# PRiME-project/PRiMEStereoMatch

Hardware: AMD Instinct MI355X
Metric: cost-volume voxels/s (CVC+CVF+WTA) (higher is better)
Workload: dtype f32; 1 GPU; synthetic 1920x1080 pair, D=256, float32 (BASELINE configs[3]); W=1920, H=1080, D=256, parallelism=1 GPU, kernel_variant=0, lr_check_on_gpu=False, batch=1, ranks=1, same_device=False, frames_in_flight=1

## Files before the change

primestereomatch_amd/csrc/psm_api_filter.cpp:

```cpp
#include "psm_ctx.h"

#include <cstring>
#include <utility>

using namespace psm;

namespace psm {

int ensure_vol(psm_ctx *c, int side)
{
    if (c->vol[side]) return 0;
    const size_t V = (size_t)c->W * c->H * c->Dloc;
    PSM_HIP(c, hipMalloc(&c->vol[side], V * velem(c)));
    return 0;
}

int ensure_ab(psm_ctx *c)
{
    if (c->ab) return 0;
    const size_t V = (size_t)c->W * c->H * c->Dloc;
    PSM_HIP(c, hipMalloc((void **)&c->ab, V * sizeof(float4)));
    return 0;
}

// ... 117 lines not shown
    sp.maps = c->Dloc == c->D && !sp.two_phase;
    sp.scratch_bytes = 2 * pc_plan_select(m, c->W, c->H, sp.n1, PC_PLANES, npairs, batch).scratch_bytes();
    return sp;
}

int enqueue_select(psm_ctx *c, const PcPairs &P, const SelPlan &sp)
{
    const bool u8 = c->dtype == PSM_U8;
    {
        Prof p(c, PSM_K_CVF_F);
        launch_cvf_select2(c->stream, c->march, P, u8, c->W, c->H, sp.n1, c->d0, next_pc_stamp(c), sp.two_phase ? 1 : 0, sp.S);
    }
    if (sp.maps && !P.tab && maps_writable(c)) return 1;
    {
        Prof p(c, PSM_K_WTA);
        launch_chunk_min2sides(c->stream, c->march, P, c->W, c->H, sp.n1, sp.maps);
    }
    if (sp.n2 > 0) {
        Prof p(c, PSM_K_CVF_F);
        launch_cvf_select_keys2(c->stream, c->march, P, u8, c->W, c->H, sp.n2, c->d0, next_pc_stamp(c), 2, sp.S);
    }
    return 0;
}

int adopt_staged_pair(psm_ctx *c)
{
    if (c->next_depth < 0) return 0;
    bool ok = true;
    if (c->range_next_pending) {
        PSM_HIP(c, hipEventSynchronize(c->ev_up));
        ok = range_inside(c, 1, -PSM_IMG_EXP, PSM_IMG_EXP);
// ... 267 lines not shown
```

primestereomatch_amd/csrc/psm_kernels.h:

```cpp
#pragma once
#include <hip/hip_runtime.h>
#include <stdint.h>

namespace psm {

struct Guidance {
    float4 *g1;
    float4 *g2;
    float4 *g3;
    float2 *g4;
};

struct March {
    int seg_rows;
    int waves;
    int flags;
    int dstep = 1;
    int inflight = 1;
    int ybeg = 0, yend = 0;
    int y0(int H) const { (void)H; return yend > ybeg ? ybeg : 0; }
    int y1(int H) const { return yend > ybeg ? yend : H; }
    int rows(int H) const { return y1(H) - y0(H); }
};

// ... 34 lines not shown
    bool narrow;
    size_t rec_per_chunk;
    int rec_bytes;
    size_t scratch_bytes() const { return rec_per_chunk * (size_t)nchunks * rec_bytes; }
};
PcPlan pc_plan(int W, int rows, int Dloc, int seg_rows_opt, int form, int batch = 1, int inflight = 1);
PcPlan pc_plan_select(March m, int W, int H, int Dloc, int form, int npairs, bool batch);
int pc_seed_stride(int W, int rows, bool u8);
constexpr int PC_TS_SLOTS = 4096;
void launch_cvf_select(hipStream_t s, March m, const float *vin, Guidance g, int W, int H, int Dloc, const float4 *g1_other,
                       int d_begin, int cvc_mode, void *scratch, unsigned long long *ts = nullptr, const uint8_t *p4_own = nullptr,
                       const uint8_t *p4_other = nullptr);
void launch_chunk_min(hipStream_t s, March m, int W, int H, int Dloc, void *scratch, long long *keys, uint8_t *map);
void launch_cvf_select2(hipStream_t s, March m, const PcPairs &P, bool u8, int W, int H, int Dloc, int d_begin, unsigned long long *ts,
                        int sel, int step);
void launch_chunk_min2sides(hipStream_t s, March m, const PcPairs &P, int W, int H, int Dloc, bool to_maps);
void launch_cvf_select_keys2(hipStream_t s, March m, const PcPairs &P, bool u8, int W, int H, int Dloc, int d_begin,
                             unsigned long long *ts, int sel, int step);
void launch_box8(hipStream_t s, int variant, March m, const float *vol, float *out, int W, int H, int Dloc);
void launch_wta(hipStream_t s, const float *vol, int W, int H, int d_begin, int Dloc, long long *keys,
                uint8_t *map);
void launch_merge(hipStream_t s, const long long *keys_all, size_t rank_stride, int nranks, int n,
                  uint8_t *map);
void launch_lr_check(hipStream_t s, const uint8_t *l, const uint8_t *r, int W, int H, uint8_t *lv,
                     uint8_t *rv);

void launch_fill_inv(hipStream_t s, uint8_t *dis, const uint8_t *valid, size_t side, int W, int H);

void launch_wgt_median(hipStream_t s, uint8_t *dis, const uint8_t *valid, const float4 *g1, int W, int H, int maxDis, int right,
                       int *nxt, int *prog, int *err);
constexpr int WM_LANE_MIN = 8192;
// ... 161 lines not shown
```

primestereomatch_amd/csrc/psm_pc.hip:

```cpp
#include "psm_kernels.h"
#include "psm_cost.h"
#include "psm_dev.h"
#include "../../include/primesm_hip.h"

#include <mutex>
#include <type_traits>

#include "psm_pc_debug.inc"

namespace psm {

typedef float f4v __attribute__((ext_vector_type(4)));

constexpr int PC_RING = 4;

template <int MODE, bool NARROW = false> struct PcLayout;
template <> struct PcLayout<0, false> { static constexpr int NA = 2, NB = 2, OUT_A = 52, OUT_B = 48, COLS = 96; };
template <> struct PcLayout<1, false> { static constexpr int NA = 2, NB = 2, OUT_A = 57, OUT_B = 54, COLS = 107; };
template <> struct PcLayout<2, false> : PcLayout<1, false> {};
template <> struct PcLayout<1, true> { static constexpr int NA = 1, NB = 1, OUT_A = 57, OUT_B = 50, COLS = 50; };
template <> struct PcLayout<2, true> : PcLayout<1, true> {};
constexpr int PC_K_LD_AUX = 0;
constexpr int PC_KEY_LD_AUX = 1;

// ... 25 lines not shown
typedef unsigned pc_u3 __attribute__((ext_vector_type(3)));
__device__ __forceinline__ float3 pc_load3(__amdgpu_buffer_rsrc_t r, int voff, int soff)
{
    const pc_u3 v = __builtin_amdgcn_raw_buffer_load_b96(r, voff, soff, 0);
    return make_float3(__uint_as_float(v.x), __uint_as_float(v.y), __uint_as_float(v.z));
}

struct PcSide {
    const float4 *G1, *G2, *G3;
    const float2 *G4;
    const float4 *Gother;
    float *kcost;
    unsigned *kdisp;
};

struct PcSel {
    int sel, step;
    int nxcd;
    int spread;
    int n;
    unsigned long long rec_total;
    int dstep;
};
__device__ __forceinline__ int pc_slice(const PcSel &o, int i)
{
    if (o.spread > 1) {
        int r = 0, base = 0;
        for (; r < o.spread; ++r) {
            const int cnt = (o.n - r + o.spread - 1) / o.spread;
            if (i < base + cnt) break;
            base += cnt;
        }
        i = (i - base) * o.spread + r;
    }
    return o.sel == 1 ? i * o.step : (o.sel == 2 ? (i / (o.step - 1)) * o.step + i % (o.step - 1) + 1 : i);
}

template <bool VEC4, int CVC, int MODE, bool U8 = false, bool BATCH = false, int VAR = 0, bool NARROW = false>
__global__ __launch_bounds__(64 * (PcLayout<MODE, NARROW>::NA + PcLayout<MODE, NARROW>::NB))
__attribute__((amdgpu_waves_per_eu(MODE == 2 ? 4 : 1, MODE == 2 ? 4 : 8)))
void k_cvf_pc(
    const float *__restrict__ vin, float *__restrict__ vout, const float4 *__restrict__ G1a, const float4 *__restrict__ G2a,
    const float4 *__restrict__ G3a, const float2 *__restrict__ G4a, int W, int H, int Dloc, int ngroups, int nsegs, int seg_rows,
    int ybeg, int yend, const float4 *__restrict__ Gothera, int d_begin, int DC, float *__restrict__ kcosta, unsigned *__restrict__ kdispa, int nbmax,
    PcSide side1, PcSel dyn, unsigned long long *__restrict__ ts, const PcPair *__restrict__ batch)
{
    constexpr bool TOL = VAR == 1, FMA = VAR == 2;
    static_assert(VAR >= 0 && VAR <= 2 && !(TOL && (U8 || MODE == 0)) && !(FMA && (U8 || BATCH)), "tolerance form: float select forms; FMA solve: float mode, single pair");
    if constexpr (BATCH) {
        static_assert(CVC == 3 && MODE != 0, "batched launches: both volumes per launch, select forms");
// ... 16 lines not shown
    const float4 *const G1 = s1 ? side1.G1 : G1a, *const G2 = s1 ? side1.G2 : G2a, *const G3 = s1 ? side1.G3 : G3a;
    const float2 *const G4 = s1 ? side1.G4 : G4a;
    const float4 *const Gother = s1 ? side1.Gother : Gothera;
    float *const kcost = s1 ? side1.kcost : kcosta;
    unsigned *const kdisp = s1 ? side1.kdisp : kdispa;
    static_assert(!NARROW || (MODE != 0 && CVC == 3), "the narrow layout exists for the two-volume select forms");
    using L = PcLayout<MODE, NARROW>;
    constexpr int PC_NA = L::NA, PC_NB = L::NB, PC_OUT_A = L::OUT_A, PC_OUT_B = L::OUT_B, PC_COLS = L::COLS;
    constexpr int PC_MCOLS = PC_NA * PC_OUT_A;
    constexpr bool SCALED = MODE != 0;
    constexpr float QSCALE = SCALED ? 0x1p-12f : 1.0f;
#define PSM_BOX(N) (SCALED ? (float)(N) : box_out(N))
    static_assert(PC_MCOLS >= PC_COLS + 7 && PC_OUT_A <= 57 && PC_OUT_B <= 57 && (MODE != 0 || (PC_COLS % 4) == 0), "bad producer/consumer layout");
    __shared__ __attribute__((aligned(16))) float4 ring[PC_RING][4][PC_MCOLS];
    __shared__ __attribute__((aligned(16))) float qbuf[MODE == 0 ? 2 : 1][MODE == 0 ? 4 : 1][MODE == 0 ? PC_COLS : 4];
    const int nchunks = (Dloc + DC - 1) / DC;
    int id = blockIdx.x;
    const int npairs = ngroups * nsegs;
    const int nitems = npairs * nchunks;
    const int ipx = (nitems + dyn.nxcd - 1) / dyn.nxcd;
    const int xcd = id % dyn.nxcd, jj = id / dyn.nxcd;
    const int item = xcd * ipx + jj;
    if (jj >= ipx || item >= nitems) return;
    if (ts != nullptr && threadIdx.x == 0) {
        (void)__hip_atomic_fetch_min(ts, (unsigned long long)wall_clock64(), __ATOMIC_RELAXED, __HIP_MEMORY_SCOPE_AGENT);
        if (blockIdx.x == 0 && blockIdx.y == 0) ts[2 * PC_TS_SLOTS] = (unsigned long long)MODE;
    }
    const int pair = item / nchunks, ch = item % nchunks;
    const int g = pair % ngroups, seg = pair / ngroups;
    const int wave = __builtin_amdgcn_readfirstlane(threadIdx.x >> 6), lane = threadIdx.x & 63;
    const bool is_a = wave < PC_NA;
    const int xg = g * PC_COLS;
    const int xm0 = xg - 4;
    const int y0 = ybeg + seg * seg_rows, y1 = min(yend, y0 + seg_rows);
    const int mstart = max(0, y0 - 4);
    const int mend = min(H - 1, max(y1 + 2, 4 - y0));
    const int nbA = (mend - mstart + 1 + 3) >> 2;
    const int nf = (y1 - y0) + 7;
    const int nbB = (nf + 3) >> 2;
    const int iters = nbB + 3;
    const int i1 = ((lane + 1) & 63) << 2, i2 = ((lane + 2) & 63) << 2, i4 = ((lane + 4) & 63) << 2;
    (void)i1;
    const size_t HW = (size_t)H * W;

    PC_TRACE_BEGIN()
    const int nds = MODE == 1 ? min(DC, Dloc - ch * DC) : 1;
    bool first = true;
    int rb = 0;
    for (int ds = 0; ds < nds; ++ds) {
    const int d = ch * DC + ds;
    const bool last_slice = ds == nds - 1;
    if (is_a) {
        const int xa0 = xm0 + wave * PC_OUT_A;
        const int ci = r101c(xa0 - 4 + lane, W);
        const int xa = xa0 + lane;
        const int xac = xa < 0 ? 0 : (xa > W - 1 ? W - 1 : xa);
        const bool mvalid = lane < PC_OUT_A;
        const float *vd = vin + (size_t)pc_slice(dyn, d) * HW;
        const int dg = d_begin + dyn.dstep * pc_slice(dyn, d);
        const bool inb = right ? (ci < W - dg) : (ci >= dg);
        const int cpart = right ? min(ci + dg, W - 1) : max(ci - dg, 0);
        const bool any_border = CVC != 0 && __builtin_amdgcn_ballot_w64(!inb) != 0;
        VTree t0 = {}, t1 = {}, t2 = {}, t3 = {};
        float pin[2];
        float4 oth[2], gin[2], o2[2], o3[2];
        float2 o4[2];
        constexpr bool LEANA = MODE == 2;
        const __amdgpu_buffer_rsrc_t rG1 = pc_rsrc(G1, (unsigned)HW * 16u), rG2 = pc_rsrc(G2, (unsigned)HW * 16u);
        const __amdgpu_buffer_rsrc_t rG3 = pc_rsrc(G3, (unsigned)HW * 16u), rG4 = pc_rsrc(G4, (unsigned)HW * 8u);
        const __amdgpu_buffer_rsrc_t rGo = pc_rsrc(CVC == 0 ? G1 : Gother, (unsigned)HW * 16u);
        const __amdgpu_buffer_rsrc_t rV = pc_rsrc(CVC == 0 ? (const void *)vd : (const void *)G1, (unsigned)HW * 4u);
        const __amdgpu_buffer_rsrc_t rPo = pc_rsrc(U8 ? (s1 ? (const void *)vin : (const void *)vout) : (const void *)G1, (unsigned)HW * 4u);
        unsigned po[2];
        const int vci = ci * 16, vcp = cpart * 16, vxa = xac * 16;
// ... 88 lines not shown
        for (int b = nbA; b < (last_slice ? iters : nbB); ++b) PC_SYNC();
#undef PSM_STEP_PA
#undef PSM_ISSUE_PA
#undef PSM_ISSUE_PIX
#undef PSM_ISSUE_GUI
#undef PSM_ISSUE_PA2
    } else {
        const int wb = wave - PC_NA;
        const int bwidth = wb < PC_NB - 1 ? PC_OUT_B : PC_COLS - (PC_NB - 1) * PC_OUT_B;
        const int xb0 = xg + wb * PC_OUT_B;
        const int xmod = xb0 - 4 + lane;
        int mc = r101(xmod, W) - xm0;
        mc = mc < 0 ? 0 : (mc > PC_MCOLS - 1 ? PC_MCOLS - 1 : mc);
        const int xb = xb0 + lane;
        const int xbc = min(xb, W - 1);
        float *od = vout + (MODE == 0 ? (size_t)pc_slice(dyn, d) * HW : 0);
        const int amax = 4 * nbA - 1;
        VTree t0 = {}, t1 = {}, t2 = {}, t3 = {};
        float o1x[4], o1y[4], o1z[4];
        const size_t krec = (size_t)(ch * npairs + pair) * nbmax * PC_COLS + wb * PC_OUT_B;
        const __amdgpu_buffer_rsrc_t rKc = pc_rsrc(MODE == 1 ? (const void *)(reinterpret_cast<float4 *>(kcost) + krec) : (const void *)G1, (unsigned)nbmax * PC_COLS * 16u);
        const __amdgpu_buffer_rsrc_t rKd = pc_rsrc(MODE == 1 ? (const void *)(kdisp + krec) : (const void *)G1, (unsigned)nbmax * PC_COLS * 4u);
#define PSM_K_LOAD(C)                                                                              \
    {                                                                                              \
        const pc_u4 v_ = __builtin_amdgcn_raw_buffer_load_b128(rKc, lane * 16, (C) * (PC_COLS * 16), PC_K_LD_AUX); \
        kq = make_float4(__uint_as_float(v_.x), __uint_as_float(v_.y), __uint_as_float(v_.z), __uint_as_float(v_.w)); \
        kd4 = __builtin_amdgcn_raw_buffer_load_b32(rKd, lane * 4, (C) * (PC_COLS * 4), PC_K_LD_AUX); \
    }
        float4 kq = make_float4(__builtin_inff(), __builtin_inff(), __builtin_inff(), __builtin_inff());
        unsigned kd4 = 0;
        long long *const keyp = reinterpret_cast<long long *>(kcost);
        const __amdgpu_buffer_rsrc_t rKy = pc_rsrc(MODE == 2 ? (const void *)keyp : (const void *)G1, (unsigned)HW * 8u);
        long long kcur[4] = {0, 0, 0, 0};
#define PSM_KEY_LOAD1(SLOT, J)                                            \
    {                                                                                              \
        int yk_ = y0 + (J) - 7;                                                                    \
        yk_ = yk_ < 0 ? 0 : (yk_ > H - 1 ? H - 1 : yk_);                                           \
        const pc_u2 v_ = __builtin_amdgcn_raw_buffer_load_b64(rKy, xbc * 8, yk_ * W * 8, PC_KEY_LD_AUX); \
        kcur[SLOT] = (long long)(((unsigned long long)v_.y << 32) | v_.x);                         \
    }
        const __amdgpu_buffer_rsrc_t rG1 = pc_rsrc(G1, (unsigned)HW * 16u);
        const int vxb = xbc * 16;
        const int dg = d_begin + dyn.dstep * pc_slice(dyn, d);
        const bool lane_out = lane < bwidth && xb < W;
#define PSM_ISSUE_PB(SLOT, J)                                                           \
    {                                                                                   \
        int yb_ = y0 + (J) - 7;                                                         \
        yb_ = yb_ < 0 ? 0 : (yb_ > H - 1 ? H - 1 : yb_);                                \
        const float3 g_ = pc_load3(rG1, vxb, yb_ * W * 16);                             \
        o1x[SLOT] = g_.x; o1y[SLOT] = g_.y; o1z[SLOT] = g_.z;                           \
    }
        auto model_of = [&](int J) -> const float4 * {
            int a = r101(y0 - 4 + J, H) - mstart;
            a = a < 0 ? 0 : (a > amax ? amax : a);
            return &ring[((a >> 2) + rb) & (PC_RING - 1)][a & 3][mc];
        };
        auto store_batch = [&](int c) {
            if constexpr (MODE == 0) {
// ... 15 lines not shown
                            if (xg + cc < W) row[cc] = src[cc];
                    }
                }
            }
            }
        };
        constexpr bool LEANB = MODE == 2;
        PSM_ISSUE_PB(0, 0) PSM_ISSUE_PB(1, 1)
        if (!LEANB) { PSM_ISSUE_PB(2, 2) PSM_ISSUE_PB(3, 3) }
        if constexpr (MODE == 1) {
            if (!first) {
                PSM_K_LOAD(0)
            }
        }
        if constexpr (MODE == 2) { PSM_KEY_LOAD1(0, 0) PSM_KEY_LOAD1(1, 1) }
        if (ds == 0) {
            PC_SYNC();
            PC_SYNC();
        }
        auto batch_b = [&](const int c) __attribute__((always_inline)) {
            if (c >= 1) store_batch(c - 1);
            {
                const int j0 = 4 * c;
                float4 a_cur = *model_of(j0), a_nxt;
                float qv[4];
#define PSM_STEP_PB(K)                                                                              \
    {                                                                                               \
        if (K < 3) a_nxt = *model_of(j0 + K + 1);      \
        double h0 = hsum8<TOL>(a_cur.x, i1, i2, i4);                                                \
        double h1 = hsum8<TOL>(a_cur.y, i1, i2, i4);                                                \
        double h2 = hsum8<TOL>(a_cur.z, i1, i2, i4);                                                \
// ... 56 lines not shown
#undef PSM_K_LOAD
    }
    if (MODE == 1) __builtin_amdgcn_s_waitcnt(0);
    first = false;
    rb = (rb + nbA) & (PC_RING - 1);
    }
#undef PSM_BOX
    if (ts != nullptr && threadIdx.x == 0)
        (void)__hip_atomic_fetch_max(ts + PC_TS_SLOTS, (unsigned long long)wall_clock64(), __ATOMIC_RELAXED, __HIP_MEMORY_SCOPE_AGENT);
    PC_TRACE_END()
}

__global__ __launch_bounds__(256) void k_chunk_min(const float4 *kcost, const unsigned *kdisp, int nchunks, int npairs,
                                                  int nbmax, int ngroups, int seg_rows, int W, int H, long long *keys,
                                                  uint8_t *map, const float4 *__restrict__ kcost1, const unsigned *__restrict__ kdisp1,
                                                  int ybeg, int yend, const PcPair *__restrict__ batch, int to_maps, int cols)
{
    if (batch) {
        const PcPair pp = batch[blockIdx.z];
        const size_t rec_total = (size_t)npairs * nbmax * cols * nchunks;
        kcost = (const float4 *)pp.scratch;
        kdisp = (const unsigned *)(kcost + rec_total);
        kcost1 = (const float4 *)((const char *)pp.scratch + rec_total * 20);
        kdisp1 = (const unsigned *)(kcost1 + rec_total);
        keys = pp.keys;
        map = to_maps ? pp.maps : nullptr;
    }
    if (blockIdx.y == 1) {
        kcost = kcost1;
        kdisp = kdisp1;
        if (keys) keys += (size_t)W * H;
        if (map) map += (size_t)W * H;
    }
    const size_t nrec = (size_t)npairs * nbmax * cols;
    const size_t idx = (size_t)blockIdx.x * blockDim.x + threadIdx.x;
    if (idx >= nrec) return;
    const int col = (int)(idx % cols);
    size_t t = idx / cols;
    const int c = (int)(t % nbmax);
    const int pair = (int)(t / nbmax);
    const int g = pair % ngroups, seg = pair / ngroups;
    const int x = g * cols + col;
    if (x >= W) return;
    const int y0 = ybeg + seg * seg_rows, y1 = min(yend, y0 + seg_rows);
    const int ya = y0 + 4 * c - 7;
    if (ya + 3 < y0 || ya >= y1) return;
    float4 kc = kcost[idx];
    unsigned kd = kdisp[idx];
    long long best[4] = {pack_key_f32(kc.x, kd & 0xff), pack_key_f32(kc.y, (kd >> 8) & 0xff), pack_key_f32(kc.z, (kd >> 16) & 0xff),
                         pack_key_f32(kc.w, kd >> 24)};
    for (int ch = 1; ch < nchunks; ++ch) {
        kc = kcost[(size_t)ch * nrec + idx];
        kd = kdisp[(size_t)ch * nrec + idx];
        const long long k0 = pack_key_f32(kc.x, kd & 0xff), k1 = pack_key_f32(kc.y, (kd >> 8) & 0xff),
                        k2 = pack_key_f32(kc.z, (kd >> 16) & 0xff), k3 = pack_key_f32(kc.w, kd >> 24);
        best[0] = k0 < best[0] ? k0 : best[0];
        best[1] = k1 < best[1] ? k1 : best[1];
        best[2] = k2 < best[2] ? k2 : best[2];
        best[3] = k3 < best[3] ? k3 : best[3];
    }
#pragma unroll
    for (int k = 0; k < 4; ++k) {
        const int yo = ya + k;
        if (yo < y0 || yo >= y1) continue;
        const size_t o = (size_t)yo * W + x;
        if (keys) keys[o] = best[k];
        if (map) map[o] = (uint8_t)((unsigned long long)best[k] & 0xffull);
    }
// ... 16 lines not shown
    int dev = 0;
    if (hipGetDevice(&dev) != hipSuccess || dev < 0 || dev >= 64) dev = 0;
    std::lock_guard<std::mutex> lock(mu);
    PcDev &d = cache[dev];
    if (d.nxcd == 0) {
        int nx = 0, cus = 0;
        if (hipDeviceGetAttribute(&nx, hipDeviceAttributeNumberOfXccs, dev) != hipSuccess || nx < 1) nx = 1;
        if (hipDeviceGetAttribute(&cus, hipDeviceAttributeMultiprocessorCount, dev) != hipSuccess || cus < 1) cus = 256;
        (void)hipGetLastError();
        d.cus_per_xcd = cus / nx > 0 ? cus / nx : 1;
        d.nxcd = nx;
    }
    return d;
}


PcPlan pc_plan(int W, int rows, int Dloc, int seg_rows_opt, int form, int batch, int inflight)
{
    const bool planes = (form & 3) == PC_PLANES, keys = (form & 3) == PC_KEYS;
    if (PSM_KNOB(planes ? "PSM_PC_SEGP" : "PSM_PC_SEGK", 0) > 0 && (planes || keys))
        seg_rows_opt = PSM_KNOB(planes ? "PSM_PC_SEGP" : "PSM_PC_SEGK", 0);
    const int sides = ((form & PC_BOTH) ? 2 : 1) * (batch > 1 ? batch : 1);
    const PcDev dev = pc_dev();
    PcPlan pl;
    pl.nxcd = dev.nxcd;
    constexpr int WIDE = PcLayout<1>::COLS, NARROW = PcLayout<1, true>::COLS;
    const bool select2 = (form & 3) != PC_STORE && (form & PC_BOTH);
    const int narrow_knob = PSM_KNOB("PSM_PC_NARROW", 0);
    pl.narrow = select2 && (narrow_knob ? narrow_knob == 1 : 2 * ((W + NARROW - 1) / NARROW) < 4 * ((W + WIDE - 1) / WIDE));
    const int cols = (form & 3) == PC_STORE ? PcLayout<0>::COLS : (pl.narrow ? NARROW : WIDE);
// ... 43 lines not shown
    pl.rec_per_chunk = (size_t)pl.ngroups * pl.nsegs * pl.nbmax * pl.cols;
    pl.rec_bytes = 20;
    return pl;
}

constexpr int PC_KEY_SPREAD = 4;

int pc_seed_stride(int W, int rows, bool u8)
{
    const int e = PSM_KNOB("PSM_PC_S", 0);
    if (e > 1) return e;
    if (rows < 200 || (u8 && (size_t)W * rows >= 1500000)) return 5;
    return 8;
}

static int pc_blocks(const PcPlan &pl, int chunks) { return pl.nxcd * ((pl.ngroups * pl.nsegs * chunks + pl.nxcd - 1) / pl.nxcd); }

struct PcArgs {
    const float *vin;
    float *vout;
    int W, H, Dloc, ybeg, yend, d_begin;
    PcSide side[2];
    PcSel sel;
    unsigned long long *ts;
    const PcPair *batch;
};

struct PcForm {
    int mode, cvc;
    bool u8;
    int var;
    bool batch, narrow, vec4;
};

template <int V> using pc_int = std::integral_constant<int, V>;
template <int... Vs, class Fn> static void pc_pick(int v, Fn &&fn) { (void)((v == Vs && (fn(pc_int<Vs>{}), true)) || ...); }
template <class Fn> static void pc_pick_bool(bool b, Fn &&fn) { if (b) fn(std::true_type{}); else fn(std::false_type{}); }

static void pc_launch(hipStream_t s, const PcPlan &pl, dim3 grid, const PcArgs &a, const PcForm &f)
{
    using F = std::false_type;
    using T = std::true_type;
    const bool planes = f.mode == PC_PLANES;
    const PcSide &s0 = a.side[0];
    auto go = [&](auto V4, auto CV, auto MD, auto U, auto BT, auto VR, auto NW) {
        using L = PcLayout<MD, NW>;
        hipLaunchKernelGGL(HIP_KERNEL_NAME(k_cvf_pc<V4, CV, MD, U, BT, VR, NW>), grid, dim3(64 * (L::NA + L::NB)), 0, s, a.vin, a.vout,
                           s0.G1, s0.G2, s0.G3, s0.G4, a.W, a.H, a.Dloc, pl.ngroups, pl.nsegs, pl.seg_rows, a.ybeg, a.yend, s0.Gother,
                           a.d_begin, planes ? pl.DC : 1, s0.kcost, s0.kdisp, planes ? pl.nbmax : 0, a.side[1], a.sel, a.ts, a.batch);
    };
    if (f.mode == PC_STORE)
        pc_pick_bool(f.vec4, [&](auto V4) { pc_pick<0, 1, 2>(f.cvc, [&](auto CV) {
            pc_pick<0, 2>(f.var, [&](auto VR) { go(V4, CV, pc_int<0>{}, F{}, F{}, VR, F{}); }); }); });
    else if (f.cvc != 3)
        pc_pick<0, 1, 2>(f.cvc, [&](auto CV) {
            if constexpr (CV != 0) if (f.u8) return go(F{}, CV, pc_int<1>{}, T{}, F{}, pc_int<0>{}, F{});
            pc_pick<0, 2>(f.var, [&](auto VR) { go(F{}, CV, pc_int<1>{}, F{}, F{}, VR, F{}); });
        });
    else
// ... 6 lines not shown

static PcSide pc_planes(const PcPlan &pl, void *scratch, int v)
{
    PcSide p = {};
    p.kcost = (float *)((char *)scratch + v * pl.scratch_bytes());
    p.kdisp = (unsigned *)(p.kcost + 4 * pl.rec_per_chunk * pl.nchunks);
    return p;
}

static int pc_var(March m, bool u8)
{
    return u8 ? 0 : (m.flags & PSM_FLAG_FMA_SOLVE) ? 2 : (m.flags & PSM_FLAG_F32_TOL) ? 1 : 0;
}

static void pc_chunk_min(hipStream_t s, March m, const PcPlan &pl, int W, int H, int sides, int npairs, void *scratch,
                         long long *keys, uint8_t *map, const PcPair *tab = nullptr, bool to_maps = false)
{
    const PcSide p0 = scratch ? pc_planes(pl, scratch, 0) : PcSide{}, p1 = scratch && sides == 2 ? pc_planes(pl, scratch, 1) : PcSide{};
    hipLaunchKernelGGL(k_chunk_min, dim3((unsigned)((pl.rec_per_chunk + 255) / 256), sides, npairs), dim3(256), 0, s,
                       (const float4 *)p0.kcost, (const unsigned *)p0.kdisp, pl.nchunks, pl.ngroups * pl.nsegs, pl.nbmax, pl.ngroups,
                       pl.seg_rows, W, H, keys, map, (const float4 *)p1.kcost, (const unsigned *)p1.kdisp, m.y0(H), m.y1(H), tab,
                       to_maps ? 1 : 0, pl.cols);
}

void launch_cvf_fused(hipStream_t s, March m, const float *vin, float *vout, Guidance gd, int W, int H, int Dloc,
                      int ybeg, int yend, const float4 *g1_other, int d_begin, int cvc_mode, unsigned long long *ts)
{
    if (yend <= ybeg) return;
    const PcPlan pl = pc_plan(W, yend - ybeg, Dloc, m.seg_rows, PC_STORE);
    PcArgs a = {vin, vout, W, H, Dloc, ybeg, yend, d_begin, {}, PcSel{0, 1, pl.nxcd, 0, Dloc, 0, 1}, ts, nullptr};
    a.side[0] = PcSide{gd.g1, gd.g2, gd.g3, gd.g4, g1_other, nullptr, nullptr};
    const int cvc = cvc_mode == 1 || cvc_mode == 2 ? cvc_mode : 0;
    pc_launch(s, pl, dim3(pc_blocks(pl, Dloc)), a, {PC_STORE, cvc, false, (m.flags & PSM_FLAG_FMA_SOLVE) ? 2 : 0, false, false, (W & 3) == 0});
}

void launch_cvf_select(hipStream_t s, March m, const float *vin, Guidance gd, int W, int H, int Dloc, const float4 *g1_other,
                       int d_begin, int cvc_mode, void *scratch, unsigned long long *ts, const uint8_t *p4_own, const uint8_t *p4_other)
{
    const PcPlan pl = pc_plan(W, m.rows(H), Dloc, m.seg_rows, PC_PLANES);
    const int cvc = cvc_mode == 1 || cvc_mode == 2 ? cvc_mode : 0;
    const bool u8 = p4_own && cvc != 0;
    PcArgs a = {u8 ? (const float *)p4_own : vin, u8 ? (float *)const_cast<uint8_t *>(p4_other) : nullptr, W, H, Dloc, m.y0(H), m.y1(H),
                d_begin, {}, PcSel{0, 1, pl.nxcd, 0, Dloc, 0, 1}, ts, nullptr};
    const PcSide k = pc_planes(pl, scratch, 0);
    a.side[0] = PcSide{gd.g1, gd.g2, gd.g3, gd.g4, g1_other, k.kcost, k.kdisp};
    pc_launch(s, pl, dim3(pc_blocks(pl, pl.nchunks)), a, {PC_PLANES, cvc, u8, (m.flags & PSM_FLAG_FMA_SOLVE) ? 2 : 0, false, false, false});
}

void launch_chunk_min(hipStream_t s, March m, int W, int H, int Dloc, void *scratch, long long *keys, uint8_t *map)
{
    pc_chunk_min(s, m, pc_plan(W, m.rows(H), Dloc, m.seg_rows, PC_PLANES), W, H, 1, 1, scratch, keys, map);
}

PcPlan pc_plan_select(March m, int W, int H, int Dloc, int form, int npairs, bool batch)
{
    return pc_plan(W, m.rows(H), Dloc, m.seg_rows, form | PC_BOTH, npairs, batch ? 1 : m.inflight);
}

static PcArgs pc_args2(March m, const PcPlan &pl, int form, const PcPairs &P, bool u8, int W, int H, int Dloc, int d_begin, PcSel sel,
                       unsigned long long *ts)
{
    PcArgs a = {nullptr, nullptr, W, H, Dloc, m.y0(H), m.y1(H), d_begin, {}, sel, ts, P.tab};
    if (P.tab) return a;
    const PcPair &p = P.one;
    if (u8) { a.vin = (const float *)p.p4[0]; a.vout = (float *)p.p4[1]; }
    for (int v = 0; v < 2; ++v) {
        const PcSide k = form == PC_PLANES ? pc_planes(pl, p.scratch, v) : PcSide{};
        a.side[v] = PcSide{p.g[v].g1, p.g[v].g2, p.g[v].g3, p.g[v].g4, p.g[v ^ 1].g1, k.kcost, k.kdisp};
        if (form == PC_KEYS) a.side[v].kcost = (float *)(p.keys + v * (size_t)W * H);
    }
    return a;
}

void launch_cvf_select2(hipStream_t s, March m, const PcPairs &P, bool u8, int W, int H, int Dloc, int d_begin, unsigned long long *ts,
                        int sel, int step)
{
    const PcPlan pl = pc_plan_select(m, W, H, Dloc, PC_PLANES, P.n, P.tab != nullptr);
    const unsigned long long rec_total = P.tab ? (unsigned long long)pl.rec_per_chunk * pl.nchunks : 0;
    const PcArgs a = pc_args2(m, pl, PC_PLANES, P, u8, W, H, Dloc, d_begin, PcSel{sel, step, pl.nxcd, 0, Dloc, rec_total, m.dstep}, ts);
    pc_launch(s, pl, dim3(pc_blocks(pl, pl.nchunks), 2, P.n), a, {PC_PLANES, 3, u8, pc_var(m, u8), P.tab != nullptr, pl.narrow, false});
}

void launch_chunk_min2sides(hipStream_t s, March m, const PcPairs &P, int W, int H, int Dloc, bool to_maps)
{
    const PcPlan pl = pc_plan_select(m, W, H, Dloc, PC_PLANES, P.n, P.tab != nullptr);
    if (P.tab) pc_chunk_min(s, m, pl, W, H, 2, P.n, nullptr, nullptr, nullptr, P.tab, to_maps);
    else pc_chunk_min(s, m, pl, W, H, 2, 1, P.one.scratch, P.one.keys, to_maps ? P.one.maps : nullptr);
}

void launch_cvf_select_keys2(hipStream_t s, March m, const PcPairs &P, bool u8, int W, int H, int Dloc, int d_begin,
                             unsigned long long *ts, int sel, int step)
{
    const PcPlan pl = pc_plan_select(m, W, H, Dloc, PC_KEYS, P.n, P.tab != nullptr);
    const PcArgs a = pc_args2(m, pl, PC_KEYS, P, u8, W, H, Dloc, d_begin,
                              PcSel{sel, step, pl.nxcd, PSM_KNOB("PSM_PC_SPREAD", PC_KEY_SPREAD), Dloc, 0, m.dstep}, ts);
    pc_launch(s, pl, dim3(pc_blocks(pl, Dloc), 2, P.n), a, {PC_KEYS, 3, u8, pc_var(m, u8), P.tab != nullptr, pl.narrow, false});
}

}
```

Baseline: 159.7 billion voxels/s.

## Skip dead disparity slices and chunks per column group in select kernels

Adds host-side liveness analysis that works out, for each column group and side, which disparity slices lie entirely outside the image border or are trivially zero. The producer/consumer select kernels and the chunk-min reduction then iterate only over live work items, with a compacted item indexing scheme and trimmed per-chunk slice ranges. This removes cost-volume filtering and reduction work for disparities that cannot affect the result. In exchange it adds index-decoding overhead in each block and falls back to full work when the live pattern is too irregular.

```diff
diff --git a/primestereomatch_amd/csrc/psm_api_filter.cpp b/primestereomatch_amd/csrc/psm_api_filter.cpp
--- a/primestereomatch_amd/csrc/psm_api_filter.cpp
+++ b/primestereomatch_amd/csrc/psm_api_filter.cpp
@@ -155,7 +155,7 @@
     if (sp.maps && !P.tab && maps_writable(c)) return 1;
     {
         Prof p(c, PSM_K_WTA);
-        launch_chunk_min2sides(c->stream, c->march, P, c->W, c->H, sp.n1, sp.maps);
+        launch_chunk_min2sides(c->stream, c->march, P, c->W, c->H, sp.n1, sp.maps, c->d0, sp.two_phase ? 1 : 0, sp.S);
     }
     if (sp.n2 > 0) {
         Prof p(c, PSM_K_CVF_F);
diff --git a/primestereomatch_amd/csrc/psm_kernels.h b/primestereomatch_amd/csrc/psm_kernels.h
--- a/primestereomatch_amd/csrc/psm_kernels.h
+++ b/primestereomatch_amd/csrc/psm_kernels.h
@@ -1,6 +1,7 @@
 #pragma once
 #include <hip/hip_runtime.h>
 #include <stdint.h>
+#include "psm_live.h"
 
 namespace psm {
 
@@ -72,7 +73,7 @@
 void launch_chunk_min(hipStream_t s, March m, int W, int H, int Dloc, void *scratch, long long *keys, uint8_t *map);
 void launch_cvf_select2(hipStream_t s, March m, const PcPairs &P, bool u8, int W, int H, int Dloc, int d_begin, unsigned long long *ts,
                         int sel, int step);
-void launch_chunk_min2sides(hipStream_t s, March m, const PcPairs &P, int W, int H, int Dloc, bool to_maps);
+void launch_chunk_min2sides(hipStream_t s, March m, const PcPairs &P, int W, int H, int Dloc, bool to_maps, int d_begin, int sel, int step);
 void launch_cvf_select_keys2(hipStream_t s, March m, const PcPairs &P, bool u8, int W, int H, int Dloc, int d_begin,
                              unsigned long long *ts, int sel, int step);
 void launch_box8(hipStream_t s, int variant, March m, const float *vol, float *out, int W, int H, int Dloc);
diff --git a/primestereomatch_amd/csrc/psm_live.h b/primestereomatch_amd/csrc/psm_live.h
--- /dev/null
+++ b/primestereomatch_amd/csrc/psm_live.h
@@ -0,0 +1,52 @@
+#pragma once
+
+#if defined(__HIPCC__)
+#define PSM_LIVE_FN __host__ __device__ inline
+#else
+#define PSM_LIVE_FN inline
+#endif
+
+namespace psm {
+
+PSM_LIVE_FN int pc_border_from(int right, int xfirst, int xlast, int W)
+{
+    if (xlast > W - 1) xlast = W - 1;
+    if (right) return (W - 1 - xfirst) + 9;
+    const int t = xlast + 7;
+    return xfirst <= 0 && t < 8 ? 8 : t;
+}
+
+PSM_LIVE_FN bool pc_dead(int right, int xfirst, int xlast, int W, int dg, int dprev)
+{
+    if (dg == 0) return true;
+    return dprev >= 0 && dprev >= pc_border_from(right, xfirst, xlast, W);
+}
+
+PSM_LIVE_FN int pc_sel_index(int sel, int step, int j)
+{
+    return sel == 1 ? j * step : (sel == 2 ? (j / (step - 1)) * step + j % (step - 1) + 1 : j);
+}
+
+struct PcOwn {
+    int on;
+    int d_begin, dstep;
+    int sel, step;
+};
+
+PSM_LIVE_FN bool pc_dead_at(const PcOwn &o, int right, int xfirst, int xlast, int W, int j)
+{
+    if (!o.on) return false;
+    const int i = pc_sel_index(o.sel, o.step, j);
+    return pc_dead(right, xfirst, xlast, W, o.d_begin + i * o.dstep, i > 0 ? o.d_begin + (i - 1) * o.dstep : -1);
+}
+
+PSM_LIVE_FN int pc_live_end(const PcOwn &o, int right, int xfirst, int xlast, int W, int n)
+{
+    if (!o.on) return n;
+    const int t = pc_border_from(right, xfirst, xlast, W);
+    const int ilim = o.d_begin >= t ? 1 : 1 + (t - o.d_begin + o.dstep - 1) / o.dstep;
+    const int below = o.sel == 1 ? (ilim + o.step - 1) / o.step : (o.sel == 2 ? ilim - (ilim + o.step - 1) / o.step : ilim);
+    return below < n ? below : n;
+}
+
+}
diff --git a/primestereomatch_amd/csrc/psm_pc.hip b/primestereomatch_amd/csrc/psm_pc.hip
--- a/primestereomatch_amd/csrc/psm_pc.hip
+++ b/primestereomatch_amd/csrc/psm_pc.hip
@@ -1,6 +1,7 @@
 #include "psm_kernels.h"
 #include "psm_cost.h"
 #include "psm_dev.h"
+#include "psm_live.h"
 #include "../../include/primesm_hip.h"
 
 #include <mutex>
@@ -63,26 +64,42 @@
     unsigned *kdisp;
 };
 
+constexpr int PC_LIVE_MAX = 6;
+struct PcLive {
+    int on;
+    int lo, full;
+    int pre[2], nshort[2], tot[2];
+    int cnt[2][PC_LIVE_MAX];
+};
+__host__ __device__ __forceinline__ int pc_live_count(const PcLive &lv, int side, int g)
+{
+    const int k = g - (side ? lv.pre[1] : lv.pre[0]), ns = side ? lv.nshort[1] : lv.nshort[0];
+    int c = lv.full;
+#pragma unroll
+    for (int i = 0; i < PC_LIVE_MAX; ++i)
+        if (i == k && i < ns) c = side ? lv.cnt[1][i] : lv.cnt[0][i];
+    return c;
+}
 struct PcSel {
     int sel, step;
     int nxcd;
     int spread;
-    int n;
     unsigned long long rec_total;
     int dstep;
+    PcLive live;
 };
-__device__ __forceinline__ int pc_slice(const PcSel &o, int i)
+__device__ __forceinline__ int pc_spread(const PcSel &o, int n, int i)
 {
     if (o.spread > 1) {
         int r = 0, base = 0;
         for (; r < o.spread; ++r) {
-            const int cnt = (o.n - r + o.spread - 1) / o.spread;
+            const int cnt = (n - r + o.spread - 1) / o.spread;
             if (i < base + cnt) break;
             base += cnt;
         }
         i = (i - base) * o.spread + r;
     }
-    return o.sel == 1 ? i * o.step : (o.sel == 2 ? (i / (o.step - 1)) * o.step + i % (o.step - 1) + 1 : i);
+    return i;
 }
 
 template <bool VEC4, int CVC, int MODE, bool U8 = false, bool BATCH = false, int VAR = 0, bool NARROW = false>
@@ -129,10 +146,11 @@
     static_assert(PC_MCOLS >= PC_COLS + 7 && PC_OUT_A <= 57 && PC_OUT_B <= 57 && (MODE != 0 || (PC_COLS % 4) == 0), "bad producer/consumer layout");
     __shared__ __attribute__((aligned(16))) float4 ring[PC_RING][4][PC_MCOLS];
     __shared__ __attribute__((aligned(16))) float qbuf[MODE == 0 ? 2 : 1][MODE == 0 ? 4 : 1][MODE == 0 ? PC_COLS : 4];
-    const int nchunks = (Dloc + DC - 1) / DC;
     int id = blockIdx.x;
     const int npairs = ngroups * nsegs;
-    const int nitems = npairs * nchunks;
+    const PcLive &lv = dyn.live;
+    const int ltot = s1 ? lv.tot[1] : lv.tot[0];
+    const int nitems = nsegs * ltot;
     const int ipx = (nitems + dyn.nxcd - 1) / dyn.nxcd;
     const int xcd = id % dyn.nxcd, jj = id / dyn.nxcd;
     const int item = xcd * ipx + jj;
@@ -141,8 +159,29 @@
         (void)__hip_atomic_fetch_min(ts, (unsigned long long)wall_clock64(), __ATOMIC_RELAXED, __HIP_MEMORY_SCOPE_AGENT);
         if (blockIdx.x == 0 && blockIdx.y == 0) ts[2 * PC_TS_SLOTS] = (unsigned long long)MODE;
     }
-    const int pair = item / nchunks, ch = item % nchunks;
-    const int g = pair % ngroups, seg = pair / ngroups;
+    const int seg = item / ltot;
+    int g, gi = item - seg * ltot, gn = lv.full;
+    {
+        const int pre = s1 ? lv.pre[1] : lv.pre[0], ns = s1 ? lv.nshort[1] : lv.nshort[0];
+        if (gi < pre * lv.full) { g = gi / lv.full; gi -= g * lv.full; }
+        else {
+            gi -= pre * lv.full;
+            g = pre;
+            bool found = false;
+#pragma unroll
+            for (int k = 0; k < PC_LIVE_MAX; ++k) {
+                const int c = s1 ? lv.cnt[1][k] : lv.cnt[0][k];
+                if (!found && k < ns) {
+                    if (gi < c) { found = true; gn = c; }
+                    else { gi -= c; ++g; }
+                }
+            }
+            if (!found) { const int q = gi / lv.full; g += q; gi -= q * lv.full; }
+        }
+    }
+    const int pair = seg * ngroups + g;
+    const int ch = lv.lo + gi;
+    const int sl0 = pc_sel_index(dyn.sel, dyn.step, MODE == 2 ? lv.lo + pc_spread(dyn, gn, gi) : ch);
     const int wave = __builtin_amdgcn_readfirstlane(threadIdx.x >> 6), lane = threadIdx.x & 63;
     const bool is_a = wave < PC_NA;
     const int xg = g * PC_COLS;
@@ -159,20 +198,26 @@
     const size_t HW = (size_t)H * W;
 
     PC_TRACE_BEGIN()
-    const int nds = MODE == 1 ? min(DC, Dloc - ch * DC) : 1;
+    int ds_lo = 0, ds_hi = MODE == 1 ? min(DC, Dloc - ch * DC) : 1;
+    if (MODE == 1 && lv.on) {
+        const PcOwn own = {1, d_begin, dyn.dstep, dyn.sel, dyn.step};
+        while (ds_lo < ds_hi && pc_dead_at(own, right, xg, xg + PC_COLS - 1, W, ch * DC + ds_lo)) ++ds_lo;
+        while (ds_hi > ds_lo && pc_dead_at(own, right, xg, xg + PC_COLS - 1, W, ch * DC + ds_hi - 1)) --ds_hi;
+        if (ds_lo >= ds_hi) return;
+    }
     bool first = true;
     int rb = 0;
-    for (int ds = 0; ds < nds; ++ds) {
-    const int d = ch * DC + ds;
-    const bool last_slice = ds == nds - 1;
+    for (int ds = ds_lo; ds < ds_hi; ++ds) {
+    const int sl = MODE == 1 ? pc_sel_index(dyn.sel, dyn.step, ch * DC + ds) : sl0;
+    const bool last_slice = ds == ds_hi - 1;
     if (is_a) {
         const int xa0 = xm0 + wave * PC_OUT_A;
         const int ci = r101c(xa0 - 4 + lane, W);
         const int xa = xa0 + lane;
         const int xac = xa < 0 ? 0 : (xa > W - 1 ? W - 1 : xa);
         const bool mvalid = lane < PC_OUT_A;
-        const float *vd = vin + (size_t)pc_slice(dyn, d) * HW;
-        const int dg = d_begin + dyn.dstep * pc_slice(dyn, d);
+        const float *vd = vin + (size_t)sl * HW;
+        const int dg = d_begin + dyn.dstep * sl;
         const bool inb = right ? (ci < W - dg) : (ci >= dg);
         const int cpart = right ? min(ci + dg, W - 1) : max(ci - dg, 0);
         const bool any_border = CVC != 0 && __builtin_amdgcn_ballot_w64(!inb) != 0;
@@ -291,7 +336,7 @@
         mc = mc < 0 ? 0 : (mc > PC_MCOLS - 1 ? PC_MCOLS - 1 : mc);
         const int xb = xb0 + lane;
         const int xbc = min(xb, W - 1);
-        float *od = vout + (MODE == 0 ? (size_t)pc_slice(dyn, d) * HW : 0);
+        float *od = vout + (MODE == 0 ? (size_t)sl * HW : 0);
         const int amax = 4 * nbA - 1;
         VTree t0 = {}, t1 = {}, t2 = {}, t3 = {};
         float o1x[4], o1y[4], o1z[4];
@@ -318,7 +363,7 @@
     }
         const __amdgpu_buffer_rsrc_t rG1 = pc_rsrc(G1, (unsigned)HW * 16u);
         const int vxb = xbc * 16;
-        const int dg = d_begin + dyn.dstep * pc_slice(dyn, d);
+        const int dg = d_begin + dyn.dstep * sl;
         const bool lane_out = lane < bwidth && xb < W;
 #define PSM_ISSUE_PB(SLOT, J)                                                           \
     {                                                                                   \
@@ -364,7 +409,7 @@
             }
         }
         if constexpr (MODE == 2) { PSM_KEY_LOAD1(0, 0) PSM_KEY_LOAD1(1, 1) }
-        if (ds == 0) {
+        if (ds == ds_lo) {
             PC_SYNC();
             PC_SYNC();
         }
@@ -451,7 +496,8 @@
 __global__ __launch_bounds__(256) void k_chunk_min(const float4 *kcost, const unsigned *kdisp, int nchunks, int npairs,
                                                   int nbmax, int ngroups, int seg_rows, int W, int H, long long *keys,
                                                   uint8_t *map, const float4 *__restrict__ kcost1, const unsigned *__restrict__ kdisp1,
-                                                  int ybeg, int yend, const PcPair *__restrict__ batch, int to_maps, int cols)
+                                                  int ybeg, int yend, const PcPair *__restrict__ batch, int to_maps, int cols,
+                                                  PcLive lv)
 {
     if (batch) {
         const PcPair pp = batch[blockIdx.z];
@@ -482,13 +528,12 @@
     const int y0 = ybeg + seg * seg_rows, y1 = min(yend, y0 + seg_rows);
     const int ya = y0 + 4 * c - 7;
     if (ya + 3 < y0 || ya >= y1) return;
-    float4 kc = kcost[idx];
-    unsigned kd = kdisp[idx];
-    long long best[4] = {pack_key_f32(kc.x, kd & 0xff), pack_key_f32(kc.y, (kd >> 8) & 0xff), pack_key_f32(kc.z, (kd >> 16) & 0xff),
-                         pack_key_f32(kc.w, kd >> 24)};
-    for (int ch = 1; ch < nchunks; ++ch) {
-        kc = kcost[(size_t)ch * nrec + idx];
-        kd = kdisp[(size_t)ch * nrec + idx];
+    const int c_lo = lv.lo, c_hi = min(nchunks, lv.lo + pc_live_count(lv, blockIdx.y == 1, g));
+    const long long none = pack_key_f32(__builtin_inff(), 0);
+    long long best[4] = {none, none, none, none};
+    for (int ch = c_lo; ch < c_hi; ++ch) {
+        const float4 kc = kcost[(size_t)ch * nrec + idx];
+        const unsigned kd = kdisp[(size_t)ch * nrec + idx];
         const long long k0 = pack_key_f32(kc.x, kd & 0xff), k1 = pack_key_f32(kc.y, (kd >> 8) & 0xff),
                         k2 = pack_key_f32(kc.z, (kd >> 16) & 0xff), k3 = pack_key_f32(kc.w, kd >> 24);
         best[0] = k0 < best[0] ? k0 : best[0];
@@ -535,6 +580,42 @@
     return d;
 }
 
+
+PcLive pc_live(int W, int cols, int ngroups, int n, int DC, bool chunks, const PcOwn &own)
+{
+    const int nu = chunks ? (n + DC - 1) / DC : n;
+    PcLive all = {};
+    all.full = nu;
+    all.tot[0] = all.tot[1] = ngroups * nu;
+    if (!own.on || n < 1 || ngroups < 1) return all;
+    PcLive lv = {};
+    lv.on = 1;
+    const int skip0 = own.d_begin == 0 && own.sel != 2 ? 1 : 0;
+    lv.lo = skip0 && (!chunks || DC == 1 || n == 1) ? 1 : 0;
+    lv.full = nu - lv.lo;
+    for (int side = 0; side < 2; ++side) {
+        int gs = -1, ge = -1;
+        for (int g = 0; g < ngroups; ++g) {
+            const int xf = g * cols, xl = xf + cols - 1;
+            const int L = pc_live_end(own, side, xf, xl, W, n);
+            if ((L < n && !pc_dead_at(own, side, xf, xl, W, L)) || (L - 1 >= skip0 && pc_dead_at(own, side, xf, xl, W, L - 1))) return all;
+            const int end = chunks ? (L + DC - 1) / DC : L, c = L > skip0 && end > lv.lo ? end - lv.lo : 0;
+            lv.tot[side] += c;
+            if (c == lv.full) continue;
+            if (gs < 0) gs = g;
+            ge = g;
+        }
+        if (gs < 0) continue;
+        if (ge - gs + 1 > PC_LIVE_MAX) return all;
+        lv.pre[side] = gs;
+        lv.nshort[side] = ge - gs + 1;
+        for (int g = gs; g <= ge; ++g) {
+            const int L = pc_live_end(own, side, g * cols, g * cols + cols - 1, W, n), end = chunks ? (L + DC - 1) / DC : L;
+            lv.cnt[side][g - gs] = L > skip0 && end > lv.lo ? end - lv.lo : 0;
+        }
+    }
+    return lv;
+}
 
 PcPlan pc_plan(int W, int rows, int Dloc, int seg_rows_opt, int form, int batch, int inflight)
 {
@@ -608,7 +689,11 @@
     return 8;
 }
 
-static int pc_blocks(const PcPlan &pl, int chunks) { return pl.nxcd * ((pl.ngroups * pl.nsegs * chunks + pl.nxcd - 1) / pl.nxcd); }
+static int pc_blocks(const PcPlan &pl, const PcLive &lv)
+{
+    const int items = pl.nsegs * (lv.tot[0] > lv.tot[1] ? lv.tot[0] : lv.tot[1]);
+    return pl.nxcd * ((items + pl.nxcd - 1) / pl.nxcd);
+}
 
 struct PcArgs {
     const float *vin;
@@ -637,6 +722,7 @@
     using T = std::true_type;
     const bool planes = f.mode == PC_PLANES;
     const PcSide &s0 = a.side[0];
+    if (grid.x == 0) return;
     auto go = [&](auto V4, auto CV, auto MD, auto U, auto BT, auto VR, auto NW) {
         using L = PcLayout<MD, NW>;
         hipLaunchKernelGGL(HIP_KERNEL_NAME(k_cvf_pc<V4, CV, MD, U, BT, VR, NW>), grid, dim3(64 * (L::NA + L::NB)), 0, s, a.vin, a.vout,
@@ -673,13 +759,13 @@
 }
 
 static void pc_chunk_min(hipStream_t s, March m, const PcPlan &pl, int W, int H, int sides, int npairs, void *scratch,
-                         long long *keys, uint8_t *map, const PcPair *tab = nullptr, bool to_maps = false)
+                         long long *keys, uint8_t *map, const PcLive &lv, const PcPair *tab = nullptr, bool to_maps = false)
 {
     const PcSide p0 = scratch ? pc_planes(pl, scratch, 0) : PcSide{}, p1 = scratch && sides == 2 ? pc_planes(pl, scratch, 1) : PcSide{};
     hipLaunchKernelGGL(k_chunk_min, dim3((unsigned)((pl.rec_per_chunk + 255) / 256), sides, npairs), dim3(256), 0, s,
                        (const float4 *)p0.kcost, (const unsigned *)p0.kdisp, pl.nchunks, pl.ngroups * pl.nsegs, pl.nbmax, pl.ngroups,
                        pl.seg_rows, W, H, keys, map, (const float4 *)p1.kcost, (const unsigned *)p1.kdisp, m.y0(H), m.y1(H), tab,
-                       to_maps ? 1 : 0, pl.cols);
+                       to_maps ? 1 : 0, pl.cols, lv);
 }
 
 void launch_cvf_fused(hipStream_t s, March m, const float *vin, float *vout, Guidance gd, int W, int H, int Dloc,
@@ -687,10 +773,11 @@
 {
     if (yend <= ybeg) return;
     const PcPlan pl = pc_plan(W, yend - ybeg, Dloc, m.seg_rows, PC_STORE);
-    PcArgs a = {vin, vout, W, H, Dloc, ybeg, yend, d_begin, {}, PcSel{0, 1, pl.nxcd, 0, Dloc, 0, 1}, ts, nullptr};
+    const PcLive lv = pc_live(W, pl.cols, pl.ngroups, Dloc, 1, false, PcOwn{});
+    PcArgs a = {vin, vout, W, H, Dloc, ybeg, yend, d_begin, {}, PcSel{0, 1, pl.nxcd, 0, 0, 1, lv}, ts, nullptr};
     a.side[0] = PcSide{gd.g1, gd.g2, gd.g3, gd.g4, g1_other, nullptr, nullptr};
     const int cvc = cvc_mode == 1 || cvc_mode == 2 ? cvc_mode : 0;
-    pc_launch(s, pl, dim3(pc_blocks(pl, Dloc)), a, {PC_STORE, cvc, false, (m.flags & PSM_FLAG_FMA_SOLVE) ? 2 : 0, false, false, (W & 3) == 0});
+    pc_launch(s, pl, dim3(pc_blocks(pl, lv)), a, {PC_STORE, cvc, false, (m.flags & PSM_FLAG_FMA_SOLVE) ? 2 : 0, false, false, (W & 3) == 0});
 }
 
 void launch_cvf_select(hipStream_t s, March m, const float *vin, Guidance gd, int W, int H, int Dloc, const float4 *g1_other,
@@ -699,18 +786,21 @@
     const PcPlan pl = pc_plan(W, m.rows(H), Dloc, m.seg_rows, PC_PLANES);
     const int cvc = cvc_mode == 1 || cvc_mode == 2 ? cvc_mode : 0;
     const bool u8 = p4_own && cvc != 0;
+    const PcLive lv = pc_live(W, pl.cols, pl.ngroups, Dloc, pl.DC, true, PcOwn{});
     PcArgs a = {u8 ? (const float *)p4_own : vin, u8 ? (float *)const_cast<uint8_t *>(p4_other) : nullptr, W, H, Dloc, m.y0(H), m.y1(H),
-                d_begin, {}, PcSel{0, 1, pl.nxcd, 0, Dloc, 0, 1}, ts, nullptr};
+                d_begin, {}, PcSel{0, 1, pl.nxcd, 0, 0, 1, lv}, ts, nullptr};
     const PcSide k = pc_planes(pl, scratch, 0);
     a.side[0] = PcSide{gd.g1, gd.g2, gd.g3, gd.g4, g1_other, k.kcost, k.kdisp};
-    pc_launch(s, pl, dim3(pc_blocks(pl, pl.nchunks)), a, {PC_PLANES, cvc, u8, (m.flags & PSM_FLAG_FMA_SOLVE) ? 2 : 0, false, false, false});
+    pc_launch(s, pl, dim3(pc_blocks(pl, lv)), a, {PC_PLANES, cvc, u8, (m.flags & PSM_FLAG_FMA_SOLVE) ? 2 : 0, false, false, false});
 }
 
 void launch_chunk_min(hipStream_t s, March m, int W, int H, int Dloc, void *scratch, long long *keys, uint8_t *map)
 {
-    pc_chunk_min(s, m, pc_plan(W, m.rows(H), Dloc, m.seg_rows, PC_PLANES), W, H, 1, 1, scratch, keys, map);
-}
-
+    const PcPlan pl = pc_plan(W, m.rows(H), Dloc, m.seg_rows, PC_PLANES);
+    pc_chunk_min(s, m, pl, W, H, 1, 1, scratch, keys, map, pc_live(W, pl.cols, pl.ngroups, Dloc, pl.DC, true, PcOwn{}));
+}
+
+static PcOwn pc_own(March m, int d_begin, int sel, int step) { return PcOwn{1, d_begin, m.dstep, sel, step}; }
 PcPlan pc_plan_select(March m, int W, int H, int Dloc, int form, int npairs, bool batch)
 {
     return pc_plan(W, m.rows(H), Dloc, m.seg_rows, form | PC_BOTH, npairs, batch ? 1 : m.inflight);
@@ -735,25 +825,73 @@
                         int sel, int step)
 {
     const PcPlan pl = pc_plan_select(m, W, H, Dloc, PC_PLANES, P.n, P.tab != nullptr);
+    const PcLive lv = pc_live(W, pl.cols, pl.ngroups, Dloc, pl.DC, true, pc_own(m, d_begin, sel, step));
     const unsigned long long rec_total = P.tab ? (unsigned long long)pl.rec_per_chunk * pl.nchunks : 0;
-    const PcArgs a = pc_args2(m, pl, PC_PLANES, P, u8, W, H, Dloc, d_begin, PcSel{sel, step, pl.nxcd, 0, Dloc, rec_total, m.dstep}, ts);
-    pc_launch(s, pl, dim3(pc_blocks(pl, pl.nchunks), 2, P.n), a, {PC_PLANES, 3, u8, pc_var(m, u8), P.tab != nullptr, pl.narrow, false});
-}
-
-void launch_chunk_min2sides(hipStream_t s, March m, const PcPairs &P, int W, int H, int Dloc, bool to_maps)
+    const PcArgs a = pc_args2(m, pl, PC_PLANES, P, u8, W, H, Dloc, d_begin, PcSel{sel, step, pl.nxcd, 0, rec_total, m.dstep, lv}, ts);
+    pc_launch(s, pl, dim3(pc_blocks(pl, lv), 2, P.n), a, {PC_PLANES, 3, u8, pc_var(m, u8), P.tab != nullptr, pl.narrow, false});
+}
+
+void launch_chunk_min2sides(hipStream_t s, March m, const PcPairs &P, int W, int H, int Dloc, bool to_maps, int d_begin, int sel, int step)
 {
     const PcPlan pl = pc_plan_select(m, W, H, Dloc, PC_PLANES, P.n, P.tab != nullptr);
-    if (P.tab) pc_chunk_min(s, m, pl, W, H, 2, P.n, nullptr, nullptr, nullptr, P.tab, to_maps);
-    else pc_chunk_min(s, m, pl, W, H, 2, 1, P.one.scratch, P.one.keys, to_maps ? P.one.maps : nullptr);
+    const PcLive lv = pc_live(W, pl.cols, pl.ngroups, Dloc, pl.DC, true, pc_own(m, d_begin, sel, step));
+    if (P.tab) pc_chunk_min(s, m, pl, W, H, 2, P.n, nullptr, nullptr, nullptr, lv, P.tab, to_maps);
+    else pc_chunk_min(s, m, pl, W, H, 2, 1, P.one.scratch, P.one.keys, to_maps ? P.one.maps : nullptr, lv);
 }
 
 void launch_cvf_select_keys2(hipStream_t s, March m, const PcPairs &P, bool u8, int W, int H, int Dloc, int d_begin,
                              unsigned long long *ts, int sel, int step)
 {
     const PcPlan pl = pc_plan_select(m, W, H, Dloc, PC_KEYS, P.n, P.tab != nullptr);
+    const PcLive lv = pc_live(W, pl.cols, pl.ngroups, Dloc, 1, false, pc_own(m, d_begin, sel, step));
     const PcArgs a = pc_args2(m, pl, PC_KEYS, P, u8, W, H, Dloc, d_begin,
-                              PcSel{sel, step, pl.nxcd, PSM_KNOB("PSM_PC_SPREAD", PC_KEY_SPREAD), Dloc, 0, m.dstep}, ts);
-    pc_launch(s, pl, dim3(pc_blocks(pl, Dloc), 2, P.n), a, {PC_KEYS, 3, u8, pc_var(m, u8), P.tab != nullptr, pl.narrow, false});
-}
-
-}
+                              PcSel{sel, step, pl.nxcd, PSM_KNOB("PSM_PC_SPREAD", PC_KEY_SPREAD), 0, m.dstep, lv}, ts);
+    pc_launch(s, pl, dim3(pc_blocks(pl, lv), 2, P.n), a, {PC_KEYS, 3, u8, pc_var(m, u8), P.tab != nullptr, pl.narrow, false});
+}
+
+}
+
+extern "C" int psm_debug_pc_dead(int right, int xfirst, int xlast, int W, int dg, int dprev)
+{
+    return psm::pc_dead(right, xfirst, xlast, W, dg, dprev) ? 1 : 0;
+}
+
+extern "C" int psm_debug_pc_items(int W, int rows, int nsl, int form, int d_begin, int dstep, int sel, int step, int *out)
+{
+    using namespace psm;
+    if (!out || W < 1 || rows < 1 || nsl < 1 || dstep < 1 || form < PC_STORE || form > PC_KEYS) return 1;
+    March m = {};
+    m.dstep = dstep;
+    m.yend = rows;
+    PcOwn own = pc_own(m, d_begin, sel, step);
+    if (form == PC_STORE) own.on = 0;
+    const PcPlan pl = form == PC_STORE ? pc_plan(W, rows, nsl, 0, PC_STORE) : pc_plan_select(m, W, rows, nsl, form, 1, false);
+    const bool chunks = form == PC_PLANES;
+    const PcLive lv = pc_live(W, pl.cols, pl.ngroups, nsl, chunks ? pl.DC : 1, chunks, own);
+    int slices[2] = {0, 0};
+    for (int side = 0; side < 2; ++side)
+        for (int g = 0; g < pl.ngroups; ++g)
+            for (int j = 0; j < nsl; ++j)
+                slices[side] += pc_dead_at(own, side, g * pl.cols, g * pl.cols + pl.cols - 1, W, j) ? 0 : 1;
+    const int v[12] = {pl.ngroups, pl.nsegs, pl.DC, pl.cols, lv.tot[0], lv.tot[1], pl.ngroups * (chunks ? pl.nchunks : nsl),
+                       slices[0], slices[1], pc_blocks(pl, lv), lv.lo, 0};
+    for (int i = 0; i < 12; ++i) out[i] = v[i];
+    return 0;
+}
+
+extern "C" int psm_debug_pc_group_items(int W, int rows, int nsl, int form, int d_begin, int dstep, int sel, int step, int side, int g,
+                                        int *out)
+{
+    using namespace psm;
+    if (!out || W < 1 || rows < 1 || nsl < 1 || dstep < 1 || form < PC_PLANES || form > PC_KEYS || side < 0 || side > 1 || g < 0) return 1;
+    March m = {};
+    m.dstep = dstep;
+    m.yend = rows;
+    const PcPlan pl = pc_plan_select(m, W, rows, nsl, form, 1, false);
+    if (g >= pl.ngroups) return 1;
+    const bool chunks = form == PC_PLANES;
+    const PcLive lv = pc_live(W, pl.cols, pl.ngroups, nsl, chunks ? pl.DC : 1, chunks, pc_own(m, d_begin, sel, step));
+    out[0] = lv.lo;
+    out[1] = pc_live_count(lv, side, g);
+    return 0;
+}
```

After: 165.2 billion voxels/s (median of 6 runs). +3.4%, better.
